# MariaPdg/thesis-fmri-reconstruction

Measured on AMD Instinct MI355X. Metric: images/sec Stage-I VAE/GAN 64x64 bs256, higher is better.
Workload: dtype f16

## Files before the change

### thesis-fmri-reconstruction_amd/csrc/api.hip

```cpp
#include "../../include/fmri_hip.h"
#include "kernels.h"
#include <stdarg.h>
#include <stdio.h>
#include <string.h>
#include <cstdlib>

using namespace fmri;

static_assert(sizeof(fmri_stat) == sizeof(StatRec) && sizeof(fmri_stat) == 32, "fmri_stat layout");
static_assert(sizeof(fmri_stat_seg) == sizeof(StatSeg) && sizeof(fmri_stat_seg) == 64, "fmri_stat_seg layout");
static_assert(FMRI_STAT_MAX_SEGS == STAT_MAX_SEGS && FMRI_STAT_BLOCKS == STAT_BLOCKS, "monitor limits");

namespace {
inline hipStream_t S(void* s) { return (hipStream_t)s; }
inline int pad_to(int v, int m) { return (v + m - 1) / m * m; }

struct TClass { int py, px, th, tw, dy0, dx0, kpad; int64_t w_off; };

void tconv_classes(int k, int pad, int ci, int rows_pad, TClass out[4]) {
    int64_t off = 0;
    for (int cy = 0; cy < 2; ++cy)
        for (int cx = 0; cx < 2; ++cx) {
            TClass& c = out[cy * 2 + cx];
            c.py = (cy + pad) & 1;
// ... 581 lines not shown
    for (int t = 0; t < k; ++t) ++nsh[(t - pad) & 1];
    int total = splits < 4 ? 4 : splits;
    total -= total & 3;
    double cost[4], csum = 0;
    for (int pl = 0; pl < 4; ++pl) { cost[pl] = 128.0 * nsh[pl >> 1] * nsh[pl & 1] + 550.0; csum += cost[pl]; }
    int smax = 1;
    for (int pl = 0; pl < 4; ++pl) {
        int sp = (int)(total * cost[pl] / csum + 0.5);
        if (sp < 1) sp = 1;
        if (sp > ntiles) sp = ntiles > 0 ? ntiles : 1;
        const int tps = (ntiles + sp - 1) / sp;
        tps_out[pl] = tps < 1 ? 1 : tps;
        const int pieces = ntiles > 0 ? (ntiles + tps_out[pl] - 1) / tps_out[pl] : 1;
        if (pieces > smax) smax = pieces;
    }
    return smax;
}

int fmri_wgrad_slabs(int N, int Yc, int Xc, int k, int pad, int splits) {
    int tps[4];
    return wgrad_plane_pieces(N, Yc, Xc, k, pad, splits, tps);
}

static int wgrad_narrow_blocks(int N, int Yc, int Xc) {
    const int64_t ntiles = (int64_t)N * ((Yc + 7) / 8) * ((Xc + 7) / 8);
    int64_t nb = (ntiles + 31) / 32;
    if (nb > 768) nb = 768;
    if (nb < 1) nb = 1;
    return (int)nb;
}
int fmri_wgrad_narrow_blocks(int N, int Yc, int Xc) {
    return (N < 1 || Yc < 1 || Xc < 1) ? 0 : wgrad_narrow_blocks(N, Yc, Xc);
}

int fmri_set_deterministic(int on) {
    const int was = g_deterministic;
    g_deterministic = on ? 1 : 0;
    return was;
}
int fmri_get_deterministic(void) { return g_deterministic; }

int fmri_wgrad(const void* P, const void* Q, float* out, const void* zero16, int N, int Yc, int Xc, int A, int Hq,
               int Wq, int Bc, int k, int stride, int pad, int flip, int apad, int ba_tile, int ldo, int splits,
               int atomic, void* stream) {
    return fmri_wgrad_if(nullptr, P, Q, out, zero16, N, Yc, Xc, A, Hq, Wq, Bc, k, stride, pad, flip, apad, ba_tile, ldo,
                         splits, atomic, stream);
}

struct WgradReq {
    const int* gate; const half_t *P, *Q, *zero; float* out;
    int N, Yc, Xc, A, Hq, Wq, Bc, k, stride, pad, flip, apad, ba_tile, ldo, splits, atomic;
    hipStream_t st;
};
static bool wgrad_win_args(const WgradReq& q, WgradWinArgs& w) {
    static const bool off = family_off("FMRI_WGRAD_WIN");
    const int64_t M = (int64_t)q.N * q.Yc * q.Xc;
    if (off || q.stride != 2 || q.flip || (q.atomic != 1 && q.atomic != 2) || q.ba_tile != 128 || (q.Bc & 31) ||
        q.Yc * q.Xc <= 1 || (int64_t)q.N * q.Hq * q.Wq * q.Bc >= 0x7fffffffLL || M * q.A >= 0x7fffffffLL)
        return false;
    for (int par = 0; par < 2; ++par) {
        int cnt = 0, emin = 0;
        for (int t = 0; t < q.k; ++t)
            if (((t - q.pad) & 1) == par) { if (!cnt) emin = t - q.pad; ++cnt; }
        if (cnt < 2 || cnt > 3) return false;
        w.nsy[par] = w.nsx[par] = cnt;
        w.tmin[par] = (emin - par) / 2;
    }
    w.gate = q.gate; w.P = q.P; w.Q = q.Q; w.out = q.out; w.zero = q.zero;
    w.N = q.N; w.Yc = q.Yc; w.Xc = q.Xc; w.A = q.A; w.Hq = q.Hq; w.Wq = q.Wq; w.Bc = q.Bc; w.pad = q.pad; w.TW = q.k;
    w.ldo = q.ldo; w.a_tiles = q.apad / 128;
    w.slab_stride = q.atomic == 2 ? (int64_t)q.apad * q.ldo : 0;
    w.tiles_y = (q.Yc + 7) / 8; w.tiles_x = (q.Xc + 7) / 8; w.ntiles = q.N * w.tiles_y * w.tiles_x;
    int tps4[4];
    const int smax = wgrad_plane_pieces(q.N, q.Yc, q.Xc, q.k, q.pad, q.splits, tps4);
    for (int pl = 0; pl < 4; ++pl) {
        w.plane_tps[pl] = tps4[pl];
        w.plane_pieces[pl] = (w.ntiles + tps4[pl] - 1) / tps4[pl];
    }
    w.splits = smax;
    w.fdTPI = make_fastdiv((uint32_t)(w.tiles_y * w.tiles_x));
    w.fdTX = make_fastdiv((uint32_t)w.tiles_x);
    return true;
}
static int wgrad_generic(const WgradReq& q) {
    WgradArgs a;
    a.gate = q.gate; a.P = q.P; a.Q = q.Q; a.out = q.out; a.zero = q.zero;
    a.N = q.N; a.Yc = q.Yc; a.Xc = q.Xc; a.A = q.A; a.Hq = q.Hq; a.Wq = q.Wq; a.Bc = q.Bc;
    a.s = q.stride; a.T = q.k * q.k; a.TW = q.k;
    a.dy0 = q.flip ? q.pad : -q.pad; a.dx0 = a.dy0; a.dstep = q.flip ? -1 : 1;
    a.M = (int)((int64_t)q.N * q.Yc * q.Xc); a.ldo = q.ldo;
    const int steps = (a.M + 63) / 64;
    const int splits = q.splits > steps ? steps : q.splits;
    a.steps_per_split = (steps + splits - 1) / splits;
    a.splits = (steps + a.steps_per_split - 1) / a.steps_per_split;
    a.atomic = q.atomic == 4 ? 2 : q.atomic;
    a.slab_stride = (int64_t)q.apad * q.ldo;
    a.ncol_chunks = a.T * q.Bc / 8;
    a.fdX = make_fastdiv((uint32_t)q.Xc);
    a.fdYX = make_fastdiv((uint32_t)(q.Yc * q.Xc));
    a.fdTW = make_fastdiv((uint32_t)q.k);
    a.fdBc8 = make_fastdiv((uint32_t)(q.Bc / 8));
    return wgrad_launch(a, q.apad, q.ba_tile, q.st);
}
static int wgrad_narrow(const WgradReq& q) {
    static const bool off = family_off("FMRI_WGRAD_NARROW");
    if (off || !(q.stride == 1 && q.k == 5 && q.pad == 2 && q.A == 32 && q.Bc == 8 && q.apad == 32 && q.Yc == q.Hq &&
                 q.Xc == q.Wq))
        return FMRI_E_UNSUPPORTED;
    if ((int64_t)q.N * q.Yc * q.Xc * 32 >= 0x7fffffffLL) return wgrad_generic(q);
    WgradNarrowArgs w;
    w.gate = q.gate; w.P = q.P; w.Q = q.Q; w.out = q.out; w.zero = q.zero;
    w.N = q.N; w.H = q.Yc; w.W = q.Xc; w.ldo = q.ldo; w.flip = q.flip;
    w.tiles_y = (q.Yc + 7) / 8; w.tiles_x = (q.Xc + 7) / 8; w.ntiles = q.N * w.tiles_y * w.tiles_x;
    w.nslabs = q.splits < 1 ? 1 : q.splits; w.pad0 = 0;
    w.slab_stride = (int64_t)q.apad * q.ldo;
    return wgrad_narrow_launch(w, wgrad_narrow_blocks(q.N, q.Yc, q.Xc), q.st);
}

int fmri_wgrad_if(const int* gate, const void* P, const void* Q, float* out, const void* zero16, int N, int Yc, int Xc,
                  int A, int Hq, int Wq, int Bc, int k, int stride, int pad, int flip, int apad, int ba_tile, int ldo,
                  int splits, int atomic, void* stream) {
    if (!P || !Q || !out || !zero16) return FMRI_E_BADARG;
    if (flip && stride != 1) return FMRI_E_UNSUPPORTED;
    if (N < 1 || A < 8 || (A & 7) || Bc < 8 || (Bc & 7) || splits < 1) return FMRI_E_BADARG;
    if (ba_tile != 32 && ba_tile != 64 && ba_tile != 128) return FMRI_E_UNSUPPORTED;
    if (apad % ba_tile || apad < A) return FMRI_E_BADARG;
    if (ldo % 128 || ldo < k * k * Bc) return FMRI_E_BADARG;
    if (splits > 1 && !atomic) return FMRI_E_BADARG;
    if (atomic < 0 || atomic > 4) return FMRI_E_BADARG;
    const int64_t M = (int64_t)N * Yc * Xc;
    if (M < 1 || M > 0x7fffff00LL) return FMRI_E_BADARG;
    const WgradReq q = {gate, (const half_t*)P, (const half_t*)Q, (const half_t*)zero16, out, N, Yc, Xc, A, Hq, Wq, Bc, k,
                        stride, pad, flip, apad, ba_tile, ldo, splits, atomic, S(stream)};
    WgradWinArgs w;
    if (wgrad_win_args(q, w)) return wgrad_win_launch(w, apad, q.st);
    if (atomic == 3) return wgrad_narrow(q);
    if (atomic == 2) return FMRI_E_UNSUPPORTED;
    return wgrad_generic(q);
}

int fmri_nchw_to_nhwc(const float* src, void* dst, int N, int C, int HW, int Cp, void* stream) {
    if (!src || !dst || (Cp & 7) || C > Cp) return FMRI_E_BADARG;
    return nchw_to_nhwc_launch(src, (half_t*)dst, N, C, HW, Cp, S(stream));
}
int fmri_nhwc_to_nchw(const void* src, float* dst, int N, int C, int HW, int Cp, float scale, void* stream) {
    if (!src || !dst || C > Cp) return FMRI_E_BADARG;
    return nhwc_to_nchw_launch((const half_t*)src, dst, N, C, HW, Cp, scale, S(stream));
}
int fmri_rows_f32_to_f16(const float* src, void* dst, int M, int C, int Cp, float scale, void* stream) {
    if (!src || !dst || C > Cp) return FMRI_E_BADARG;
    return rows_f32_to_f16_launch(src, (half_t*)dst, M, C, Cp, scale, S(stream));
}
int fmri_rows_f16_to_f32(const void* src, float* dst, int M, int C, int Cp, float scale, void* stream) {
    if (!src || !dst || C > Cp) return FMRI_E_BADARG;
    return rows_f16_to_f32_launch((const half_t*)src, dst, M, C, Cp, scale, S(stream));
}
int fmri_reduce_slabs(const float* slabs, int nslabs, int64_t slab_stride, int M, int C, int ld, const float* bias,
                      int act, float* out32, int ld32, void* out16, int ld16, void* stream) {
    if (!slabs || nslabs < 1 || C > ld) return FMRI_E_BADARG;
    return reduce_slabs_launch(slabs, nslabs, slab_stride, M, C, ld, bias, act, out32, ld32, (half_t*)out16, ld16,
                               S(stream));
}
int fmri_permute_chw(const float* src, float* dst, int C, int HW, int to_engine, float scale, int accumulate,
                     void* stream) {
    if (!src || !dst) return FMRI_E_BADARG;
    return permute_chw_launch(src, dst, C, HW, to_engine, scale, accumulate, S(stream));
}

int64_t fmri_bn_ws_floats(int M, int C) { return (M < 1 || C < 8) ? 0 : bn_ws_floats(M, C); }

int fmri_bn_stats(const void* x, int M, int C, float* sums2C, float* ws, int64_t ws_floats, void* stream) {
    if (!x || !sums2C || (C & 7) || M < 1) return FMRI_E_BADARG;
    return bn_stats_launch((const half_t*)x, M, C, sums2C, ws, ws_floats, S(stream));
}
int fmri_bn_finalize(const float* sums2C, int C, float count, const float* gamma, const float* beta, float eps,
                     float momentum, int updates, float* running_mean, float* running_var, float* mean, float* rstd,
                     float* scale, float* shift, int64_t* num_batches_tracked, void* stream) {
    if (!sums2C || !gamma || !beta || !mean || !rstd || !scale || !shift) return FMRI_E_BADARG;
    return bn_finalize_launch(sums2C, C, count, gamma, beta, eps, momentum, updates, running_mean, running_var, mean,
                              rstd, scale, shift, (long long*)num_batches_tracked, nullptr, S(stream));
}
int fmri_bn_finalize_s(const float* sums2C, int C, float count, const float* gamma, const float* beta, float eps,
                       float momentum, int updates, float* running_mean, float* running_var, float* mean, float* rstd,
                       float* scale, float* shift, int64_t* num_batches_tracked, const float* in_scale, void* stream) {
    if (!sums2C || !gamma || !beta || !mean || !rstd || !scale || !shift) return FMRI_E_BADARG;
    return bn_finalize_launch(sums2C, C, count, gamma, beta, eps, momentum, updates, running_mean, running_var, mean,
                              rstd, scale, shift, (long long*)num_batches_tracked, in_scale, S(stream));
}
int fmri_bn_stats_finalize(const void* x, int M, int C, float* sums2C, float* ws, int64_t ws_floats, float count,
                           const float* gamma, const float* beta, float eps, float momentum, int updates,
                           float* running_mean, float* running_var, float* mean, float* rstd, float* scale,
                           float* shift, int64_t* num_batches_tracked, void* stream) {
    if (!x || !sums2C || (C & 7) || M < 1 || !gamma || !beta || !mean || !rstd || !scale || !shift)
        return FMRI_E_BADARG;
    return bn_stats_finalize_launch((const half_t*)x, M, C, sums2C, ws, ws_floats, count, gamma, beta, eps, momentum,
                                    updates, running_mean, running_var, mean, rstd, scale, shift,
                                    (long long*)num_batches_tracked, S(stream));
}
int fmri_bn_cols_fwd(const void* x, void* y, int M, int C, float count, const float* gamma, const float* beta, float eps,
                     float momentum, int updates, float* running_mean, float* running_var, float* mean, float* rstd,
                     float* scale, float* shift, float* sums2C, int64_t* num_batches_tracked, int relu, void* stream) {
    if (!x || !y || !sums2C || (C & 7) || C < 8 || M < 1 || !gamma || !beta || !mean || !rstd || !scale || !shift)
        return FMRI_E_BADARG;
    return bn_cols_fwd_launch((const half_t*)x, (half_t*)y, M, C, count, gamma, beta, eps, momentum, updates, running_mean,
                              running_var, mean, rstd, scale, shift, sums2C, (long long*)num_batches_tracked, relu,
                              nullptr, S(stream));
}
int fmri_bn_cols_fwd_s(const void* x, void* y, int M, int C, float count, const float* gamma, const float* beta, float eps,
                       float momentum, int updates, float* running_mean, float* running_var, float* mean, float* rstd,
                       float* scale, float* shift, float* sums2C, int64_t* num_batches_tracked, int relu,
                       const float* in_scale, void* stream) {
    if (!x || !y || !sums2C || (C & 7) || C < 8 || M < 1 || !gamma || !beta || !mean || !rstd || !scale || !shift)
        return FMRI_E_BADARG;
    return bn_cols_fwd_launch((const half_t*)x, (half_t*)y, M, C, count, gamma, beta, eps, momentum, updates, running_mean,
                              running_var, mean, rstd, scale, shift, sums2C, (long long*)num_batches_tracked, relu,
                              in_scale, S(stream));
}
int fmri_bn_cols_bwd(const void* x, const void* dy, void* dx, int M, int C, int nstreams, float count, const float* mean,
// ... 301 lines not shown
```

### thesis-fmri-reconstruction_amd/csrc/kernels.h

```cpp
#pragma once
#include "common.h"

namespace fmri {

struct PackArgs {
    const float* src;
    half_t* dst;
    int64_t sa, sta, sb, stb;
    int32_t A, TA, B, Bp;
    int32_t KW, py, px, step, TH, TW;
    int32_t rows_pad, kpad;
};

struct PackEntry {
    PackArgs p;
    int32_t run;
    int32_t tile_begin;
};

struct UnpackArgs {
    const float* src;
    float* dst;
    int64_t sa, sta, sb, stb;
    int32_t A, TA, B, Bp;
// ... 40 lines not shown
    int32_t nonfinite, clamped, written;
};
struct StatSeg {
    const float* x;
    int64_t rows, cols, ld;
    const float* div;
    const int* gate;
    StatRec* out;
    float scale, clamp;
};
constexpr int STAT_MAX_SEGS = 8, STAT_BLOCKS = 256;
struct StatSegs {
    StatSeg s[STAT_MAX_SEGS];
    int32_t nblk[STAT_MAX_SEGS];
};
int apply_batch_stats_launch(const ApplyEntry* tab, int n, int total_tiles, const ApplyOpt& o, StatRec* part,
                             hipStream_t st);
int stat_fold_launch(const StatRec* part, int nrec, const int* flag, StatRec* out, hipStream_t st);
int tensor_stats_launch(const StatSegs& segs, int nseg, StatRec* ws, hipStream_t st);

struct StatAcc {
    double ss;
    float mx, mn, amax;
    int nf, cl;
};
__device__ __forceinline__ void stat_init(StatAcc& a) {
    a.ss = 0.0; a.mx = -__builtin_inff(); a.mn = __builtin_inff(); a.amax = 0.f; a.nf = 0; a.cl = 0;
}
__device__ __forceinline__ void stat_add(StatAcc& a, float v) {
    if (__builtin_isfinite(v)) {
        a.ss += (double)v * (double)v;
        a.mx = fmaxf(a.mx, v); a.mn = fminf(a.mn, v); a.amax = fmaxf(a.amax, fabsf(v));
    } else {
        a.nf += 1;
    }
}
__device__ __forceinline__ void stat_add_clamped(StatAcc& a, float v, float clamp) {
    stat_add(a, v);
    if (clamp > 0.f) a.cl += fminf(fmaxf(v, -clamp), clamp) != v ? 1 : 0;
}
__device__ __forceinline__ void stat_merge(StatAcc& a, const StatAcc& b) {
    a.ss += b.ss; a.mx = fmaxf(a.mx, b.mx); a.mn = fminf(a.mn, b.mn); a.amax = fmaxf(a.amax, b.amax);
    a.nf += b.nf; a.cl += b.cl;
}
__device__ __forceinline__ void stat_merge_rec(StatAcc& a, const StatRec& r) {
    a.ss += r.sumsq; a.mx = fmaxf(a.mx, r.max); a.mn = fminf(a.mn, r.min); a.amax = fmaxf(a.amax, r.max_abs);
    a.nf += r.nonfinite; a.cl += r.clamped;
}
__device__ __forceinline__ StatRec stat_rec(const StatAcc& a, int written) {
    StatRec r;
    r.sumsq = a.ss; r.max = a.mx; r.min = a.mn; r.max_abs = a.amax; r.nonfinite = a.nf; r.clamped = a.cl;
    r.written = written;
    return r;
}
__device__ __forceinline__ StatAcc stat_block(StatAcc a, StatAcc* red) {
#pragma unroll
    for (int o = 32; o > 0; o >>= 1) {
        a.ss += __shfl_xor(a.ss, o, 64);
        a.mx = fmaxf(a.mx, __shfl_xor(a.mx, o, 64));
        a.mn = fminf(a.mn, __shfl_xor(a.mn, o, 64));
        a.amax = fmaxf(a.amax, __shfl_xor(a.amax, o, 64));
        a.nf += __shfl_xor(a.nf, o, 64);
        a.cl += __shfl_xor(a.cl, o, 64);
    }
    __syncthreads();
    if ((threadIdx.x & 63) == 0) red[threadIdx.x >> 6] = a;
    __syncthreads();
    StatAcc r = red[0];
    for (int w = 1; w < (int)(blockDim.x >> 6); ++w) stat_merge(r, red[w]);
    return r;
}

int igemm_launch(const IgemmArgs& a, int maxM, int bn_tile, int copad, bool out_f32, hipStream_t st);
int igemm_bm(const IgemmArgs& a, int maxM, int bn_tile, int copad, bool out_f32);
int igemm_tc32_launch(const Tc32Args& a, int nblocks, hipStream_t st);
int igemm_tc5_launch(const Tc5Args& a, int bn_tile, int copad, hipStream_t st);
int igemm_c5_launch(const C5Args& a, int copad, hipStream_t st);
int igemm_c5w_launch(const C5Args& a, int copad, hipStream_t st);
int igemm_tc5w_launch(const Tc5Args& a, int copad, hipStream_t st);
int mlp_fwd_launch(const MlpFwdArgs& a, hipStream_t st);
int mlp_bwd_launch(const MlpBwdArgs& a, hipStream_t st);
int igemm_narrow_launch(const NarrowArgs& a, int ci, int co_tiles, bool flip, hipStream_t st);
int wgrad_launch(const WgradArgs& a, int apad, int ba_tile, hipStream_t st);
int wgrad_win_launch(const WgradWinArgs& a, int apad, hipStream_t st);
int wgrad_narrow_launch(const WgradNarrowArgs& a, int nblocks, hipStream_t st);

int pack_weight_launch(const PackArgs& p, hipStream_t st);
int unpack_grad_launch(const UnpackArgs& p, hipStream_t st);
int pack_tile_count(const PackArgs& p, int* run_out);
int pack_batch_launch(const PackEntry* tab, int n, int total_tiles, hipStream_t st);
struct TransposeEntry {
    const half_t* src;
    half_t* dst;
    int32_t R, C, Rbuf;
    int32_t width;
    int32_t lds, ldd;
    int32_t tile_begin, pad_;
};
int transpose_batch_launch(const TransposeEntry* tab, int n, int total_tiles, hipStream_t st);
int transpose_f16_launch(const half_t* src, half_t* dst, int R, int C, int Rbuf, int lds_, int ldd, hipStream_t st);
int nchw_to_nhwc_launch(const float* s, half_t* d, int N, int C, int HW, int Cp, hipStream_t st);
int nhwc_to_nchw_launch(const half_t* s, float* d, int N, int C, int HW, int Cp, float scale, hipStream_t st);
int rows_f32_to_f16_launch(const float* s, half_t* d, int M, int C, int Cp, float scale, hipStream_t st);
int rows_f16_to_f32_launch(const half_t* s, float* d, int M, int C, int Cp, float scale, hipStream_t st);
int reduce_slabs_launch(const float* slabs, int nslabs, int64_t slab_stride, int M, int C, int ld, const float* bias,
                        int act, float* out32, int ld32, half_t* out16, int ld16, hipStream_t st);
int permute_chw_launch(const float* s, float* d, int C, int HW, int to_engine, float scale, int accumulate,
                       hipStream_t st);

int64_t bn_ws_floats(int M, int C);
int bn_stats_launch(const half_t* x, int M, int C, float* sums, float* ws, int64_t ws_floats, hipStream_t st);
int bn_bwd_reduce2_launch(const half_t* x, const half_t* dy, int M, int C, const float* mean, const float* rstd,
                          const float* gamma, const float* beta, int relu, float* sums4C, float* ws, int64_t ws_floats,
                          float* dbeta, float* dgamma, float gscale, int param_stream, hipStream_t st);
int bn_bwd_apply2_launch(const half_t* x, const half_t* dy, half_t* dx, int M, int C, float count, const float* mean,
                         const float* rstd, const float* gamma, const float* beta, int relu, const float* sums4C,
                         int* cnt, hipStream_t st);
int bn_stats_finalize_launch(const half_t* x, int M, int C, float* sums, float* ws, int64_t ws_floats, float count,
                             const float* gamma, const float* beta, float eps, float momentum, int updates, float* rm,
                             float* rv, float* mean, float* rstd, float* scale, float* shift, long long* nbt,
                             hipStream_t st);
int bn_bwd_reduce_launch(const half_t* x, const half_t* dy, int M, int C, const float* mean, const float* rstd,
                         const float* gamma, const float* beta, int relu, float* sums, float* ws, int64_t ws_floats,
                         float* dbeta, float* dgamma, float gscale, hipStream_t st);
constexpr int FOLD_STAGE_ROWS = 32;
int bn_fold_finalize_launch(const float* part, int rows, int C, float* scratch, float* sums, float count,
                            const float* gamma, const float* beta, float eps, float momentum, int updates, float* rm,
                            float* rv, float* mean, float* rstd, float* scale, float* shift, long long* nbt,
                            hipStream_t st);
int bn_fold_launch(const float* part, int rows, int n, float* scratch, float* sums, hipStream_t st);
int bn_bwd_fold_launch(const float* part, int rows, int rows_cap, int C, int G, float* scratch, float* sums,
                       float* dbeta, float* dgamma, float gscale, int pgroup, hipStream_t st);
int bn_finalize_launch(const float* sums, int C, float count, const float* gamma, const float* beta, float eps,
                       float momentum, int updates, float* rm, float* rv, float* mean, float* rstd, float* scale,
                       float* shift, long long* nbt, const float* in_scale, hipStream_t st);
int bn_cols_fwd_launch(const half_t* x, half_t* y, int M, int C, float count, const float* gamma, const float* beta,
                       float eps, float momentum, int updates, float* rm, float* rv, float* mean, float* rstd,
                       float* scale, float* shift, float* sums2C, long long* nbt, int relu, const float* in_scale,
                       hipStream_t st);
int bn_cols_bwd_launch(const half_t* x, const half_t* dy, half_t* dx, int M, int C, int nstreams, float count,
                       const float* mean, const float* rstd, const float* gamma, const float* beta, int relu, float* sums,
                       float* dbeta, float* dgamma, float gscale, int pstream, int* cnt, hipStream_t st);
int bn_apply_launch(const half_t* x, half_t* y, int M, int C, const float* scale, const float* shift, int relu,
                    hipStream_t st);
int bn_bwd_apply_launch(const half_t* x, const half_t* dy, half_t* dx, int M, int C, float count, const float* mean,
                        const float* rstd, const float* gamma, const float* beta, int relu, const float* sums,
                        int* cnt, hipStream_t st);
int act_bwd_launch(const half_t* y, const half_t* dy, half_t* dpre, int M, int C, int act, float* colsum, float* ws,
                   int64_t ws_floats, float* dbias, int dbias_n, float gscale, hipStream_t st);
int colsum_rows_launch(const half_t* x, int M, int C, float* sums2C, float* ws, int64_t ws_floats, float* dbias,
                       int dbias_n, float gscale, hipStream_t st);
int colsum_acc_launch(const void* src, int is_f16, int M, int C, int64_t ld_row, int64_t ld_col, float scale, float* dst,
                      hipStream_t st);

bool route_probe(const char* fmt, ...);

extern int g_deterministic;

int latent_fwd_launch(const float* head, const float* eps, int B, int Z, int zp, half_t* z16, float* kl_rows,
                      float* kl_total, int sample, hipStream_t st);
int latent_ranged_launch(const float* head, const float* eps, int B, int Z, int zp, half_t* z16, float* kl_rows,
                         float* kl_total, int sample, float* z32, float* zmax, float* zscale, float cap, int phase,
                         hipStream_t st);
int rows_absmax_launch(const float* x, int64_t n, float* zmax, hipStream_t st);
float latent_range_scale_host(float zmax, float cap);
int latent_bwd_launch(const float* head, const float* eps, const float* dz, int ldz, float dz_unscale, float kl_w,
                      const float* kl_dev, int B, int Z, float out_scale, half_t* dhead16, float* dhead32, int sample,
// ... 55 lines not shown
```

### thesis-fmri-reconstruction_amd/csrc/wgrad_win.hip

```cpp
#include "kernels.h"
#include "pipe.h"

namespace fmri {


template <int NSY, int NSX, bool SLABS>
__device__ __forceinline__ void wgrad_win_body(const WgradWinArgs& a, char* smem, int py, int px, int a_tile,
                                               int b_tile, int split) {
    constexpr int WH = 8 + NSY - 1, WW = 8 + NSX - 1;
    constexpr int P_BYTES = 64 * 256;
    constexpr int W_BYTES = ((WH * WW * 64 + 1023) / 1024) * 1024;
    constexpr int STAGE = P_BYTES + W_BYTES;
    constexpr int NS = NSY * NSX;
    constexpr int TA = 4;

    const int lane = threadIdx.x & 63;
    const int wave_all = __builtin_amdgcn_readfirstlane(threadIdx.x >> 6);
    const bool loader = wave_all >= 4;
    const int wave = wave_all & 3;
    const int tid = threadIdx.x & 255;
    const int a0 = a_tile * 128;
    const int b0 = b_tile * 32;
    const int tminy = a.tmin[py], tminx = a.tmin[px];

    const int trow = tid >> 4;
    const int cphys = tid & 15;
    const int fsw = (((trow & 3) | (((trow >> 3) & 1) << 2)) << 1);
    const int clog = cphys ^ fsw;
    const bool p_on = a0 + clog * 8 < a.A;
    const int prow = trow >> 3, pcol = trow & 7;
    const uint32_t lane_p = (uint32_t)(((prow * a.Xc + pcol) * a.A + a0 + clog * 8) * 2);

    int wj[2], wi[2];
    bool won[2];
    uint32_t lane_q[2];
#pragma unroll
    for (int e = 0; e < 2; ++e) {
        const int u = tid + 256 * e;
        const int pix = u >> 2;
        won[e] = pix < WH * WW;
        wj[e] = pix / WW;
        wi[e] = pix - wj[e] * WW;
        lane_q[e] = (uint32_t)(((2 * wj[e] * a.Wq + 2 * wi[e]) * a.Bc + b0 + (tid & 3) * 8) * 2);
    }
    const v4i srdP = make_srd(a.P, (uint32_t)a.N * (uint32_t)a.Yc * (uint32_t)a.Xc * (uint32_t)a.A * 2u);
    const v4i srdQ = make_srd(a.Q, (uint32_t)a.N * (uint32_t)a.Hq * (uint32_t)a.Wq * (uint32_t)a.Bc * 2u);

    const int tps = a.plane_tps[py * 2 + px];
    const int t0 = split * tps;
    int t1 = t0 + tps;
    if (t1 > a.ntiles) t1 = a.ntiles;
    const int nsteps = t1 > t0 ? t1 - t0 : 0;
    if (nsteps == 0 && a.slab_stride == 0) return;
    const int tpi = a.tiles_y * a.tiles_x;

    int kYc = a.Yc, kXc = a.Xc, kA = a.A, kHq = a.Hq, kWq = a.Wq, kBc = a.Bc, ktx = a.tiles_x, ktpi = tpi;
    uint32_t tpi_magic = a.fdTPI.magic, tpi_sh = a.fdTPI.sh, tx_magic = a.fdTX.magic, tx_sh = a.fdTX.sh;
    FMRI_KEEP(kYc); FMRI_KEEP(kXc); FMRI_KEEP(kA); FMRI_KEEP(kHq); FMRI_KEEP(kWq); FMRI_KEEP(kBc); FMRI_KEEP(ktx);
    FMRI_KEEP(ktpi); FMRI_KEEP(tpi_magic); FMRI_KEEP(tpi_sh); FMRI_KEEP(tx_magic); FMRI_KEEP(tx_sh);
    const FastDiv fTPI{tpi_magic, tpi_sh, 0, 0}, fTX{tx_magic, tx_sh, 0, 0};
    const uint32_t lds0 = (uint32_t)(uintptr_t)smem;
    const uint32_t prow_step = (uint32_t)(2 * kXc * kA * 2);

    auto stage_load = [&](int buf, int t) __attribute__((always_inline)) {
        const int n = (int)fd_div((uint32_t)t, fTPI);
        const int trem = t - n * ktpi;
        const int tyi = (int)fd_div((uint32_t)trem, fTX);
        const int txi = trem - tyi * ktx;
        const int y0 = tyi * 8, x0 = txi * 8;
        const uint32_t tile_p = (uint32_t)(((n * kYc + y0) * kXc + x0) * kA * 2);
        const bool pcol_ok = p_on && x0 + pcol < kXc;
        const uint32_t dstP = lds0 + buf * STAGE + wave * (4 * 256);
#pragma unroll
        for (int i = 0; i < 4; ++i) {
            const bool ok = pcol_ok && y0 + prow + 2 * i < kYc;
            bdma16(srdP, ok ? tile_p + lane_p + i * prow_step : 0x80000000u, dstP + i * (16 * 256));
        }
        const int by = 2 * (y0 + tminy) + py, bx = 2 * (x0 + tminx) + px;
        const int tile_q = ((n * kHq + by) * kWq + bx) * kBc * 2;
        const uint32_t dstW = lds0 + buf * STAGE + P_BYTES + wave * 1024;
#pragma unroll
        for (int e = 0; e < 2; ++e) {
            if (e * 4096 + wave * 1024 < W_BYTES) {
                const int iy = by + 2 * wj[e], ix = bx + 2 * wi[e];
                const bool ok = won[e] && (unsigned)iy < (unsigned)kHq && (unsigned)ix < (unsigned)kWq;
                bdma16(srdQ, ok ? (uint32_t)(tile_q + (int)lane_q[e]) : 0x80000000u, dstW + e * 4096);
            }
        }
    };

    f4 acc[NS][TA];
#pragma unroll
    for (int s = 0; s < NS; ++s)
#pragma unroll
        for (int i = 0; i < TA; ++i) acc[s][i] = (f4){0.f, 0.f, 0.f, 0.f};

    const int wa = wave >> 1, wb = wave & 1;
    const int g = lane >> 4, q = (lane >> 2) & 3, p = lane & 3;
    const int fr = ((q | ((g & 1) << 2)) << 1);
    const int rowoff = (8 * g + q) * 256 + (p & 1) * 8;
    const int woff = (g * WW + q) * 64 + wb * 32 + p * 8;

    auto compute = [&](int buf) {
        const char* Ps = smem + buf * STAGE;
        const char* Ws = Ps + P_BYTES + woff;
        constexpr int NI = 2 * NS;
        auto read_a = [&](int ks, int ta) __attribute__((always_inline)) -> h8 {
            const int blk = wa * 4 + ta;
            const int ch = (2 * blk + (p >> 1)) ^ fr;
            const char* ad = Ps + ks * (32 * 256) + rowoff + ch * 16;
            union { s4v s[2]; h8 h; } u;
            u.s[0] = __builtin_amdgcn_ds_read_tr16_b64_v4i16((__attribute__((address_space(3))) s4v*)(ad));
            u.s[1] = __builtin_amdgcn_ds_read_tr16_b64_v4i16((__attribute__((address_space(3))) s4v*)(ad + 4 * 256));
            return u.h;
        };
        auto read_w = [&](int i) __attribute__((always_inline)) -> h8 {
            const int ks = i / NS, sh = i % NS, sy = sh / NSX, sx = sh % NSX;
            const char* ad = Ws + ((ks * 4 + sy) * WW + sx) * 64;
            union { s4v s[2]; h8 h; } u;
            u.s[0] = __builtin_amdgcn_ds_read_tr16_b64_v4i16((__attribute__((address_space(3))) s4v*)(ad));
            u.s[1] = __builtin_amdgcn_ds_read_tr16_b64_v4i16((__attribute__((address_space(3))) s4v*)(ad + 4 * 64));
            return u.h;
        };
        h8 af[2][TA], wf[3];
#pragma unroll
        for (int ta = 0; ta < TA; ++ta) af[0][ta] = read_a(0, ta);
        wf[0] = read_w(0);
        wf[1] = read_w(1);
        __builtin_amdgcn_sched_barrier(0);
        static_for<0, NI>([&](auto I_) __attribute__((always_inline)) {
            constexpr int i = decltype(I_)::value;
            constexpr int ks = i / NS, sh = i % NS;
            constexpr bool rd_w = i + 2 < NI, rd_a = i >= NS - TA && i < NS;
            if constexpr (rd_w) wf[(i + 2) % 3] = read_w(i + 2);
            if constexpr (rd_a) af[1][i - (NS - TA)] = read_a(1, i - (NS - TA));
#pragma unroll
            for (int ta = 0; ta < TA; ++ta)
                acc[sh][ta] = SLABS ? __builtin_amdgcn_mfma_f32_16x16x32_f16(wf[i % 3], af[ks][ta], acc[sh][ta], 0, 0, 0)
                                    : __builtin_amdgcn_mfma_f32_16x16x32_f16(af[ks][ta], wf[i % 3], acc[sh][ta], 0, 0, 0);
            if constexpr (rd_w || rd_a) __builtin_amdgcn_sched_group_barrier(0x100, (rd_w ? 2 : 0) + (rd_a ? 2 : 0), 0);
            __builtin_amdgcn_sched_group_barrier(0x008, TA, 0);
        });
        __builtin_amdgcn_sched_barrier(0);
    };

    if (loader) {
        const bool short_wave = 4096 + wave * 1024 >= W_BYTES;
        if (nsteps > 0) stage_load(0, t0);
        if (nsteps > 1) stage_load(1, t0 + 1);
        int nxt = 2;
        for (int it = 0; it < nsteps; ++it) {
            if (it + 1 < nsteps) {
                if (short_wave) asm volatile("s_waitcnt vmcnt(5)" ::: "memory");
                else asm volatile("s_waitcnt vmcnt(6)" ::: "memory");
            } else {
                asm volatile("s_waitcnt vmcnt(0)" ::: "memory");
            }
            __builtin_amdgcn_s_barrier();
            __builtin_amdgcn_sched_barrier(0);
            if (it + 2 < nsteps) stage_load(nxt, t0 + it + 2);
            if (++nxt == 3) nxt = 0;
        }
        return;
    }
    int cur = 0;
    for (int it = 0; it < nsteps; ++it) {
        asm volatile("s_waitcnt lgkmcnt(0)" ::: "memory");
        __builtin_amdgcn_s_barrier();
        __builtin_amdgcn_sched_barrier(0);
        compute(cur);
        if (++cur == 3) cur = 0;
    }

    int kldo = a.ldo, kpad = a.pad, kTW = a.TW;
    float* slab = a.out + (int64_t)split * a.slab_stride;
    FMRI_KEEP(kldo); FMRI_KEEP(kpad); FMRI_KEEP(kTW); FMRI_KEEP(slab);
    const int bcol = b0 + wb * 16 + (SLABS ? (lane >> 4) * 4 : (lane & 15));
    if (bcol >= kBc) return;
    const int nfill = (SLABS && split + 1 == a.plane_pieces[py * 2 + px]) ? a.splits - split : 1;
#pragma unroll
    for (int sy = 0; sy < NSY; ++sy)
#pragma unroll
        for (int sx = 0; sx < NSX; ++sx) {
            const int ty = 2 * (tminy + sy) + py + kpad;
            const int tx = 2 * (tminx + sx) + px + kpad;
            const int col = (ty * kTW + tx) * kBc + bcol;
#pragma unroll
            for (int ta = 0; ta < TA; ++ta) {
                const f4 v = acc[sy * NSX + sx][ta];
                if constexpr (SLABS) {
                    const int arow = a0 + wa * 64 + ta * 16 + (lane & 15);
                    *(f4*)(slab + (int64_t)arow * kldo + col) = v;
                    for (int sl = 1; sl < nfill; ++sl)
                        *(f4*)(slab + sl * a.slab_stride + (int64_t)arow * kldo + col) = (f4){0.f, 0.f, 0.f, 0.f};
                } else {
                    const int arow = a0 + wa * 64 + ta * 16 + (lane >> 4) * 4;
#pragma unroll
                    for (int r = 0; r < 4; ++r) atomicAdd(slab + (int64_t)(arow + r) * kldo + col, v[r]);
                }
            }
        }
}

template <bool SLABS>
__global__ __launch_bounds__(512, 1) void wgrad_win_kernel(const WgradWinArgs a) {
    if (a.gate && *a.gate == 0) return;
    extern __shared__ __attribute__((aligned(16))) char smem[];
    const int nb = gridDim.x;
    int logical = blockIdx.x;
    if ((nb & 7) == 0) logical = (logical & 7) * (nb >> 3) + (logical >> 3);
    const int nbt = a.Bc >> 5;
    const int groups = nbt * a.a_tiles;
    int piece = logical / groups;
    int rem = logical - piece * groups;
    const int b_tile = rem % nbt;
    const int a_tile = rem / nbt;
    int plane = 0;
    while (plane < 3 && piece >= a.plane_pieces[plane]) { piece -= a.plane_pieces[plane]; ++plane; }
    const int split = piece;
    const int py = plane >> 1, px = plane & 1;
    const int nsy = a.nsy[py], nsx = a.nsx[px];
    if (nsy == 3 && nsx == 3) wgrad_win_body<3, 3, SLABS>(a, smem, py, px, a_tile, b_tile, split);
    else if (nsy == 3 && nsx == 2) wgrad_win_body<3, 2, SLABS>(a, smem, py, px, a_tile, b_tile, split);
    else if (nsy == 2 && nsx == 3) wgrad_win_body<2, 3, SLABS>(a, smem, py, px, a_tile, b_tile, split);
    else wgrad_win_body<2, 2, SLABS>(a, smem, py, px, a_tile, b_tile, split);
}

int wgrad_win_launch(const WgradWinArgs& a, int apad, hipStream_t st) {
    if ((int64_t)a.N * a.Yc * a.Xc * a.A * 2 >= 0x80000000LL || (int64_t)a.N * a.Hq * a.Wq * a.Bc * 2 >= 0x80000000LL)
        return E_UNSUPPORTED;
    dim3 grid((a.Bc / 32) * a.a_tiles * (a.plane_pieces[0] + a.plane_pieces[1] + a.plane_pieces[2] + a.plane_pieces[3]));
    const int lds = 3 * (64 * 256 + 7 * 1024);
    if (hipFuncSetAttribute((const void*)wgrad_win_kernel<true>, hipFuncAttributeMaxDynamicSharedMemorySize, lds) != hipSuccess) return E_LAUNCH;
    if (hipFuncSetAttribute((const void*)wgrad_win_kernel<false>, hipFuncAttributeMaxDynamicSharedMemorySize, lds) != hipSuccess) return E_LAUNCH;
    if (a.slab_stride != 0) hipLaunchKernelGGL(wgrad_win_kernel<true>, grid, dim3(512), lds, st, a);
    else hipLaunchKernelGGL(wgrad_win_kernel<false>, grid, dim3(512), lds, st, a);
    return hipGetLastError() == hipSuccess ? OK : E_LAUNCH;
}


}
```

Before: 39170.

## Process two tiles per pipeline interval in windowed wgrad kernel

The windowed weight-gradient kernel now loads and computes two 8x8 tiles per pipeline stage (TPS=2), doubling LDS per stage and halving the number of barrier-synchronised iterations. The MFMA loop runs over both tiles' A and W fragments in one unrolled sequence, and an odd trailing tile is handled separately. The aim is to amortise barrier and waitcnt overhead and give longer MFMA runs between syncs. The cost is triple the stage LDS footprint (about 140KB), more vmcnt outstanding, and more register pressure. It is enabled whenever any plane has at least two tiles per piece, and an env var can force the old behaviour.

```diff
diff --git a/thesis-fmri-reconstruction_amd/csrc/api.hip b/thesis-fmri-reconstruction_amd/csrc/api.hip
--- a/thesis-fmri-reconstruction_amd/csrc/api.hip
+++ b/thesis-fmri-reconstruction_amd/csrc/api.hip
@@ -687,6 +687,13 @@
     w.fdTX = make_fastdiv((uint32_t)w.tiles_x);
     return true;
 }
+static int wgrad_win_tps(const WgradWinArgs& w) {
+    static const bool one = [] { const char* v = getenv("FMRI_WW_TPS"); return v && !strcmp(v, "1"); }();
+    if (one) return 1;
+    for (int pl = 0; pl < 4; ++pl)
+        if (w.plane_tps[pl] >= 2) return 2;
+    return 1;
+}
 static int wgrad_generic(const WgradReq& q) {
     WgradArgs a;
     a.gate = q.gate; a.P = q.P; a.Q = q.Q; a.out = q.out; a.zero = q.zero;
@@ -738,7 +745,7 @@
     const WgradReq q = {gate, (const half_t*)P, (const half_t*)Q, (const half_t*)zero16, out, N, Yc, Xc, A, Hq, Wq, Bc, k,
                         stride, pad, flip, apad, ba_tile, ldo, splits, atomic, S(stream)};
     WgradWinArgs w;
-    if (wgrad_win_args(q, w)) return wgrad_win_launch(w, apad, q.st);
+    if (wgrad_win_args(q, w)) return wgrad_win_launch(w, apad, wgrad_win_tps(w), q.st);
     if (atomic == 3) return wgrad_narrow(q);
     if (atomic == 2) return FMRI_E_UNSUPPORTED;
     return wgrad_generic(q);
diff --git a/thesis-fmri-reconstruction_amd/csrc/kernels.h b/thesis-fmri-reconstruction_amd/csrc/kernels.h
--- a/thesis-fmri-reconstruction_amd/csrc/kernels.h
+++ b/thesis-fmri-reconstruction_amd/csrc/kernels.h
@@ -146,7 +146,7 @@
 int mlp_bwd_launch(const MlpBwdArgs& a, hipStream_t st);
 int igemm_narrow_launch(const NarrowArgs& a, int ci, int co_tiles, bool flip, hipStream_t st);
 int wgrad_launch(const WgradArgs& a, int apad, int ba_tile, hipStream_t st);
-int wgrad_win_launch(const WgradWinArgs& a, int apad, hipStream_t st);
+int wgrad_win_launch(const WgradWinArgs& a, int apad, int tiles_per_interval, hipStream_t st);
 int wgrad_narrow_launch(const WgradNarrowArgs& a, int nblocks, hipStream_t st);
 
 int pack_weight_launch(const PackArgs& p, hipStream_t st);
diff --git a/thesis-fmri-reconstruction_amd/csrc/wgrad_win.hip b/thesis-fmri-reconstruction_amd/csrc/wgrad_win.hip
--- a/thesis-fmri-reconstruction_amd/csrc/wgrad_win.hip
+++ b/thesis-fmri-reconstruction_amd/csrc/wgrad_win.hip
@@ -4,13 +4,14 @@
 namespace fmri {
 
 
-template <int NSY, int NSX, bool SLABS>
+template <int NSY, int NSX, bool SLABS, int TPS>
 __device__ __forceinline__ void wgrad_win_body(const WgradWinArgs& a, char* smem, int py, int px, int a_tile,
                                                int b_tile, int split) {
     constexpr int WH = 8 + NSY - 1, WW = 8 + NSX - 1;
     constexpr int P_BYTES = 64 * 256;
     constexpr int W_BYTES = ((WH * WW * 64 + 1023) / 1024) * 1024;
-    constexpr int STAGE = P_BYTES + W_BYTES;
+    constexpr int SLOT = P_BYTES + W_BYTES;
+    constexpr int STAGE = TPS * SLOT;
     constexpr int NS = NSY * NSX;
     constexpr int TA = 4;
 
@@ -46,9 +47,9 @@
     const v4i srdP = make_srd(a.P, (uint32_t)a.N * (uint32_t)a.Yc * (uint32_t)a.Xc * (uint32_t)a.A * 2u);
     const v4i srdQ = make_srd(a.Q, (uint32_t)a.N * (uint32_t)a.Hq * (uint32_t)a.Wq * (uint32_t)a.Bc * 2u);
 
-    const int tps = a.plane_tps[py * 2 + px];
-    const int t0 = split * tps;
-    int t1 = t0 + tps;
+    const int piece_tiles = a.plane_tps[py * 2 + px];
+    const int t0 = split * piece_tiles;
+    int t1 = t0 + piece_tiles;
     if (t1 > a.ntiles) t1 = a.ntiles;
     const int nsteps = t1 > t0 ? t1 - t0 : 0;
     if (nsteps == 0 && a.slab_stride == 0) return;
@@ -62,7 +63,7 @@
     const uint32_t lds0 = (uint32_t)(uintptr_t)smem;
     const uint32_t prow_step = (uint32_t)(2 * kXc * kA * 2);
 
-    auto stage_load = [&](int buf, int t) __attribute__((always_inline)) {
+    auto stage_load = [&](int slot, int t) __attribute__((always_inline)) {
         const int n = (int)fd_div((uint32_t)t, fTPI);
         const int trem = t - n * ktpi;
         const int tyi = (int)fd_div((uint32_t)trem, fTX);
@@ -70,7 +71,7 @@
         const int y0 = tyi * 8, x0 = txi * 8;
         const uint32_t tile_p = (uint32_t)(((n * kYc + y0) * kXc + x0) * kA * 2);
         const bool pcol_ok = p_on && x0 + pcol < kXc;
-        const uint32_t dstP = lds0 + buf * STAGE + wave * (4 * 256);
+        const uint32_t dstP = lds0 + slot + wave * (4 * 256);
 #pragma unroll
         for (int i = 0; i < 4; ++i) {
             const bool ok = pcol_ok && y0 + prow + 2 * i < kYc;
@@ -78,7 +79,7 @@
         }
         const int by = 2 * (y0 + tminy) + py, bx = 2 * (x0 + tminx) + px;
         const int tile_q = ((n * kHq + by) * kWq + bx) * kBc * 2;
-        const uint32_t dstW = lds0 + buf * STAGE + P_BYTES + wave * 1024;
+        const uint32_t dstW = lds0 + slot + P_BYTES + wave * 1024;
 #pragma unroll
         for (int e = 0; e < 2; ++e) {
             if (e * 4096 + wave * 1024 < W_BYTES) {
@@ -101,22 +102,23 @@
     const int rowoff = (8 * g + q) * 256 + (p & 1) * 8;
     const int woff = (g * WW + q) * 64 + wb * 32 + p * 8;
 
-    auto compute = [&](int buf) {
-        const char* Ps = smem + buf * STAGE;
+    auto compute = [&](int stage, auto NT_) {
+        constexpr int NT = decltype(NT_)::value;
+        const char* Ps = smem + stage * STAGE;
         const char* Ws = Ps + P_BYTES + woff;
-        constexpr int NI = 2 * NS;
-        auto read_a = [&](int ks, int ta) __attribute__((always_inline)) -> h8 {
+        constexpr int NI = 2 * NS, NJ = NT * NI;
+        auto read_a = [&](int h, int ta) __attribute__((always_inline)) -> h8 {
             const int blk = wa * 4 + ta;
             const int ch = (2 * blk + (p >> 1)) ^ fr;
-            const char* ad = Ps + ks * (32 * 256) + rowoff + ch * 16;
+            const char* ad = Ps + (h >> 1) * SLOT + (h & 1) * (32 * 256) + rowoff + ch * 16;
             union { s4v s[2]; h8 h; } u;
             u.s[0] = __builtin_amdgcn_ds_read_tr16_b64_v4i16((__attribute__((address_space(3))) s4v*)(ad));
             u.s[1] = __builtin_amdgcn_ds_read_tr16_b64_v4i16((__attribute__((address_space(3))) s4v*)(ad + 4 * 256));
             return u.h;
         };
-        auto read_w = [&](int i) __attribute__((always_inline)) -> h8 {
-            const int ks = i / NS, sh = i % NS, sy = sh / NSX, sx = sh % NSX;
-            const char* ad = Ws + ((ks * 4 + sy) * WW + sx) * 64;
+        auto read_w = [&](int j) __attribute__((always_inline)) -> h8 {
+            const int i = j % NI, ks = i / NS, sh = i % NS, sy = sh / NSX, sx = sh % NSX;
+            const char* ad = Ws + (j / NI) * SLOT + ((ks * 4 + sy) * WW + sx) * 64;
             union { s4v s[2]; h8 h; } u;
             u.s[0] = __builtin_amdgcn_ds_read_tr16_b64_v4i16((__attribute__((address_space(3))) s4v*)(ad));
             u.s[1] = __builtin_amdgcn_ds_read_tr16_b64_v4i16((__attribute__((address_space(3))) s4v*)(ad + 4 * 64));
@@ -128,48 +130,62 @@
         wf[0] = read_w(0);
         wf[1] = read_w(1);
         __builtin_amdgcn_sched_barrier(0);
-        static_for<0, NI>([&](auto I_) __attribute__((always_inline)) {
+        static_for<0, NJ>([&](auto I_) __attribute__((always_inline)) {
             constexpr int i = decltype(I_)::value;
-            constexpr int ks = i / NS, sh = i % NS;
-            constexpr bool rd_w = i + 2 < NI, rd_a = i >= NS - TA && i < NS;
+            constexpr int h = i / NS, sh = i % NS;
+            constexpr bool rd_w = i + 2 < NJ, rd_a = sh >= NS - TA && h + 1 < 2 * NT;
             if constexpr (rd_w) wf[(i + 2) % 3] = read_w(i + 2);
-            if constexpr (rd_a) af[1][i - (NS - TA)] = read_a(1, i - (NS - TA));
+            if constexpr (rd_a) af[(h + 1) & 1][sh - (NS - TA)] = read_a(h + 1, sh - (NS - TA));
 #pragma unroll
             for (int ta = 0; ta < TA; ++ta)
-                acc[sh][ta] = SLABS ? __builtin_amdgcn_mfma_f32_16x16x32_f16(wf[i % 3], af[ks][ta], acc[sh][ta], 0, 0, 0)
-                                    : __builtin_amdgcn_mfma_f32_16x16x32_f16(af[ks][ta], wf[i % 3], acc[sh][ta], 0, 0, 0);
+                acc[sh][ta] = SLABS ? __builtin_amdgcn_mfma_f32_16x16x32_f16(wf[i % 3], af[h & 1][ta], acc[sh][ta], 0, 0, 0)
+                                    : __builtin_amdgcn_mfma_f32_16x16x32_f16(af[h & 1][ta], wf[i % 3], acc[sh][ta], 0, 0, 0);
             if constexpr (rd_w || rd_a) __builtin_amdgcn_sched_group_barrier(0x100, (rd_w ? 2 : 0) + (rd_a ? 2 : 0), 0);
             __builtin_amdgcn_sched_group_barrier(0x008, TA, 0);
         });
         __builtin_amdgcn_sched_barrier(0);
     };
 
+    const int nint = (nsteps + TPS - 1) / TPS;
     if (loader) {
         const bool short_wave = 4096 + wave * 1024 >= W_BYTES;
-        if (nsteps > 0) stage_load(0, t0);
-        if (nsteps > 1) stage_load(1, t0 + 1);
+        auto interval_load = [&](int stage, int i) __attribute__((always_inline)) {
+            stage_load(stage * STAGE, t0 + TPS * i);
+            if (TPS == 2 && 2 * i + 1 < nsteps) stage_load(stage * STAGE + SLOT, t0 + 2 * i + 1);
+        };
+        if (nint > 0) interval_load(0, 0);
+        if (nint > 1) interval_load(1, 1);
         int nxt = 2;
-        for (int it = 0; it < nsteps; ++it) {
-            if (it + 1 < nsteps) {
-                if (short_wave) asm volatile("s_waitcnt vmcnt(5)" ::: "memory");
-                else asm volatile("s_waitcnt vmcnt(6)" ::: "memory");
+        for (int it = 0; it < nint; ++it) {
+            if (it + 1 >= nint) {
+                wait_vmcnt<0>();
+            } else if (TPS == 2 && 2 * it + 3 < nsteps) {
+                if (short_wave) wait_vmcnt<10>();
+                else wait_vmcnt<12>();
             } else {
-                asm volatile("s_waitcnt vmcnt(0)" ::: "memory");
+                if (short_wave) wait_vmcnt<5>();
+                else wait_vmcnt<6>();
             }
             __builtin_amdgcn_s_barrier();
             __builtin_amdgcn_sched_barrier(0);
-            if (it + 2 < nsteps) stage_load(nxt, t0 + it + 2);
+            if (it + 2 < nint) interval_load(nxt, it + 2);
             if (++nxt == 3) nxt = 0;
         }
         return;
     }
     int cur = 0;
-    for (int it = 0; it < nsteps; ++it) {
+    for (int it = 0; it < nsteps / TPS; ++it) {
         asm volatile("s_waitcnt lgkmcnt(0)" ::: "memory");
         __builtin_amdgcn_s_barrier();
         __builtin_amdgcn_sched_barrier(0);
-        compute(cur);
+        compute(cur, std::integral_constant<int, TPS>{});
         if (++cur == 3) cur = 0;
+    }
+    if (TPS == 2 && (nsteps & 1)) {
+        asm volatile("s_waitcnt lgkmcnt(0)" ::: "memory");
+        __builtin_amdgcn_s_barrier();
+        __builtin_amdgcn_sched_barrier(0);
+        compute(cur, std::integral_constant<int, 1>{});
     }
 
     int kldo = a.ldo, kpad = a.pad, kTW = a.TW;
@@ -202,7 +218,7 @@
         }
 }
 
-template <bool SLABS>
+template <bool SLABS, int TPS>
 __global__ __launch_bounds__(512, 1) void wgrad_win_kernel(const WgradWinArgs a) {
     if (a.gate && *a.gate == 0) return;
     extern __shared__ __attribute__((aligned(16))) char smem[];
@@ -220,23 +236,29 @@
     const int split = piece;
     const int py = plane >> 1, px = plane & 1;
     const int nsy = a.nsy[py], nsx = a.nsx[px];
-    if (nsy == 3 && nsx == 3) wgrad_win_body<3, 3, SLABS>(a, smem, py, px, a_tile, b_tile, split);
-    else if (nsy == 3 && nsx == 2) wgrad_win_body<3, 2, SLABS>(a, smem, py, px, a_tile, b_tile, split);
-    else if (nsy == 2 && nsx == 3) wgrad_win_body<2, 3, SLABS>(a, smem, py, px, a_tile, b_tile, split);
-    else wgrad_win_body<2, 2, SLABS>(a, smem, py, px, a_tile, b_tile, split);
-}
-
-int wgrad_win_launch(const WgradWinArgs& a, int apad, hipStream_t st) {
+    if (nsy == 3 && nsx == 3) wgrad_win_body<3, 3, SLABS, TPS>(a, smem, py, px, a_tile, b_tile, split);
+    else if (nsy == 3 && nsx == 2) wgrad_win_body<3, 2, SLABS, TPS>(a, smem, py, px, a_tile, b_tile, split);
+    else if (nsy == 2 && nsx == 3) wgrad_win_body<2, 3, SLABS, TPS>(a, smem, py, px, a_tile, b_tile, split);
+    else wgrad_win_body<2, 2, SLABS, TPS>(a, smem, py, px, a_tile, b_tile, split);
+}
+
+template <bool SLABS, int TPS>
+static int launch_as(const WgradWinArgs& a, dim3 grid, hipStream_t st) {
+    const int lds = 3 * TPS * (64 * 256 + 7 * 1024);
+    if (hipFuncSetAttribute((const void*)wgrad_win_kernel<SLABS, TPS>, hipFuncAttributeMaxDynamicSharedMemorySize, lds) != hipSuccess)
+        return E_LAUNCH;
+    hipLaunchKernelGGL((wgrad_win_kernel<SLABS, TPS>), grid, dim3(512), lds, st, a);
+    return hipGetLastError() == hipSuccess ? OK : E_LAUNCH;
+}
+
+int wgrad_win_launch(const WgradWinArgs& a, int apad, int tiles_per_interval, hipStream_t st) {
     if ((int64_t)a.N * a.Yc * a.Xc * a.A * 2 >= 0x80000000LL || (int64_t)a.N * a.Hq * a.Wq * a.Bc * 2 >= 0x80000000LL)
         return E_UNSUPPORTED;
     dim3 grid((a.Bc / 32) * a.a_tiles * (a.plane_pieces[0] + a.plane_pieces[1] + a.plane_pieces[2] + a.plane_pieces[3]));
-    const int lds = 3 * (64 * 256 + 7 * 1024);
-    if (hipFuncSetAttribute((const void*)wgrad_win_kernel<true>, hipFuncAttributeMaxDynamicSharedMemorySize, lds) != hipSuccess) return E_LAUNCH;
-    if (hipFuncSetAttribute((const void*)wgrad_win_kernel<false>, hipFuncAttributeMaxDynamicSharedMemorySize, lds) != hipSuccess) return E_LAUNCH;
-    if (a.slab_stride != 0) hipLaunchKernelGGL(wgrad_win_kernel<true>, grid, dim3(512), lds, st, a);
-    else hipLaunchKernelGGL(wgrad_win_kernel<false>, grid, dim3(512), lds, st, a);
-    return hipGetLastError() == hipSuccess ? OK : E_LAUNCH;
-}
-
-
-}
+    const bool two = tiles_per_interval == 2;
+    if (a.slab_stride != 0) return two ? launch_as<true, 2>(a, grid, st) : launch_as<true, 1>(a, grid, st);
+    return two ? launch_as<false, 2>(a, grid, st) : launch_as<false, 1>(a, grid, st);
+}
+
+
+}
```

Result: no change. 39150 (-0.0%).
